# JubSteven/POEM-v2

Hardware: AMD Instinct MI355X
Metric: samples/sec (multi-view frames) POEM-medium 8-view (higher is better)
Workload: dtype f32

## Files before the change

poem-v2_amd/csrc/decoder.cpp:

```cpp
#include "engine.h"

int build_anchor_tables(poem_handle_t h, Plan& p, hipStream_t s, bool at_create) {
  const poem_config_t& c = h->cfg;
  const int C = c.embed, Q = c.nquery;
  const bool ov = !at_create && h->overlap && h->bps_stream && h->knn_stream;
  hipStream_t sk = ov ? h->knn_stream : s;
  if (ov) {
    HIPCHK(hipEventRecord(h->ev_fork0, s));
    HIPCHK(hipStreamWaitEvent(sk, h->ev_fork0, 0));
  }
  const int bb0 = h->block_base(0);
  HIPCHK(poem_launch_canon_xyz(h->tmpl, p.canon_xyz, Q * 3, c.radius, sk));
  for (int k = 0; k < 2; ++k) {
    const int vb = bb0 + (k == 0 ? B_VS : B_VC);
    HIPCHK(poem_launch_vector_attention_tables(p.canon_xyz, h->anchor, h->anchor_idx, h->R(vb + 4), h->R(vb + 5),
                                               h->P(vb + 6), h->R(vb + 7), h->fused[0].w[5 + k], p.tab_g[k], p.tab_p[k],
                                               Q, C, sk));
  }
  if (ov) HIPCHK(hipEventRecord(h->ev_tab, sk));
  h->tables_pending = ov;
  return POEM_OK;
}

namespace {

struct DecoderRun {
  poem_handle_t h;
  Plan& p;
  const poem_config_t& c;
  const float *pt_xyz, *pt_feats;
  float *pose_aa, *betas;
  const int B, C, S, Q, BS, BQ;
// ... 251 lines not shown
      const auto& sw = h->split[2 * i];
      HIPCHK(poem_launch_vector_attention_split(xyz, xyz, anchor, idx_s, shared, p.y3, p.y3 + C, p.y3 + 2 * C, Q, h->R(vsb + 4),
                                                h->R(vsb + 5), sw.w[0], h->R(vsb + 7), sw.w[1], sw.w[2], sw.scales, p.rs, B, Q, C,
                                                3 * C, 3 * C, 3 * C, s));
    } else if (tables && i == 0) {
      if (ov && h->tables_pending) HIPCHK(hipStreamWaitEvent(s, h->ev_tab, 0));
      if (anchor_from_y3)
        HIPCHK(poem_launch_vector_attention_anchored(h->anchor_idx, p.y3, p.y3 + C, p.y3 + 2 * C, Q, h->P(vsb + 10), p.tab_g[0], p.tab_p[0],
                                                     p.rs, B, Q, C, 3 * C, 3 * C, 3 * C, s));
      else {
      if (ov) HIPCHK(hipStreamWaitEvent(s, h->ev_xyz[0], 0));
      HIPCHK(poem_launch_vector_attention_anchored(p.ident, p.y3, p.anch_kv[0], p.anch_kv[0] + C, 32, h->P(vsb + 10), p.tab_g[0],
                                                   p.tab_p[0], p.rs, B, Q, C, 3 * C, 2 * C, 2 * C, s));
      }
    } else if (!shared && p.idx_ld != 32) {
      HIPCHK(poem_launch_vector_attention_k(xyz, xyz, idx_s, kq, p.idx_ld, p.y3, p.y3 + C, p.y3 + 2 * C, Q, h->R(vsb + 4), h->R(vsb + 5),
                                            h->P(vsb + 6), h->R(vsb + 7), h->fused[i].w[5], h->R(vsb + 9), h->P(vsb + 10), h->R(vsb + 11),
                                            p.rs, B, Q, C, 3 * C, 3 * C, 3 * C, 1, s));
    } else {
      poem_vecattn_one_query_blocks(h->va_p1);
      poem_vecattn_valid_neighbours(kq);
      const hipError_t ve = poem_launch_vector_attention(xyz, xyz, anchor, idx_s, shared, p.y3, p.y3 + C, p.y3 + 2 * C, Q, h->R(vsb + 4),
                                                         h->R(vsb + 5), h->P(vsb + 6), h->R(vsb + 7), h->fused[i].w[5], h->R(vsb + 9),
                                                         h->P(vsb + 10), h->R(vsb + 11), p.rs, B, Q, C, 3 * C, 3 * C, 3 * C, 1, s);
      poem_vecattn_valid_neighbours(32);
      poem_vecattn_one_query_blocks(0);
      HIPCHK(ve);
    }
    if (const int rc = prof_end(prof, tables && i == 0 ? 1 : 0); rc != POEM_OK) return rc;
    if (chain) {
      ChainArgs cc = chain_args(1);
      cc.x = p.rs; cc.ldx = C;
      cc.w1 = (const float4*)h->P(vsb + 2); cc.b1 = h->R(vsb + 3); cc.res = hidden; cc.ldres = C; cc.res_mod = 0;
      cc.y1 = p.f_self[i]; cc.ldy1 = C;
      cc.w2 = (const float4*)h->fused[i].w[4]; cc.b2 = h->fused[i].b[4]; cc.n2 = 1; cc.y2 = p.qc; cc.ldy2 = C;
      HIPCHK(poem_launch_chain(&cc, C, s));
      return POEM_OK;
    }
    if (const int rc = gemm(p.rs, C, vsb + 2, vsb + 3, hidden, C, p.f_self[i], C, BQ, C, C, POEM_ACT_NONE); rc != POEM_OK) return rc;
    HIPCHK(poem_launch_gemm(p.f_self[i], C, h->fused[i].w[4], h->fused[i].b[4], nullptr, 0, p.qc, C, BQ, C, C, POEM_ACT_NONE, s));
    return POEM_OK;
// ... 8 lines not shown
        bps_waited[k] = true;
      }
    const bool prof = prof_begin();
    const int kc = shared ? 32 : c.knn;
    if (h->precision != POEM_PRECISION_FP32) {
      if (kc != 32) return POEM_E_UNSUPPORTED;
      const auto& sw = h->split[2 * i + 1];
      HIPCHK(poem_launch_vector_attention_split(xyz, pt_xyz_rows, anchor, idx_c, shared, p.qc, p.y1[i] + 4 * (size_t)BSP * C,
                                                p.y1[i] + 5 * (size_t)BSP * C, SP, h->R(vcb + 4), h->R(vcb + 5), sw.w[0],
                                                h->R(vcb + 7), sw.w[1], sw.w[2], sw.scales, p.rc, B, Q, C, C, C, C, s));
    } else if (tables && i == 0) {
      if (ov) HIPCHK(hipStreamWaitEvent(s, h->ev_xyz[0], 0));
      HIPCHK(poem_launch_vector_attention_anchored(p.ident, p.qc, p.anch_kv[1], p.anch_kv[1] + C, 32, h->P(vcb + 10), p.tab_g[1],
                                                   p.tab_p[1], p.rc, B, Q, C, C, 2 * C, 2 * C, s));
    } else if (!shared && p.idx_ld != 32) {
      HIPCHK(poem_launch_vector_attention_k(xyz, pt_xyz_rows, idx_c, kc, p.idx_ld, p.qc, p.y1[i] + 4 * (size_t)BSP * C, p.y1[i] + 5 * (size_t)BSP * C,
                                            SP, h->R(vcb + 4), h->R(vcb + 5), h->P(vcb + 6), h->R(vcb + 7), h->fused[i].w[6], h->R(vcb + 9),
                                            h->P(vcb + 10), h->R(vcb + 11), p.rc, B, Q, C, C, C, C, 1, s));
    } else {
      poem_vecattn_one_query_blocks(h->va_p1);
      poem_vecattn_valid_neighbours(kc);
      const hipError_t ve = poem_launch_vector_attention(xyz, pt_xyz_rows, anchor, idx_c, shared, p.qc, p.y1[i] + 4 * (size_t)BSP * C,
                                                         p.y1[i] + 5 * (size_t)BSP * C, SP, h->R(vcb + 4), h->R(vcb + 5), h->P(vcb + 6),
                                                         h->R(vcb + 7), h->fused[i].w[6], h->R(vcb + 9), h->P(vcb + 10), h->R(vcb + 11), p.rc, B,
                                                         Q, C, C, C, C, 1, s);
      poem_vecattn_valid_neighbours(32);
      poem_vecattn_one_query_blocks(0);
      HIPCHK(ve);
    }
    return prof_end(prof, tables && i == 0 ? 1 : 0);
  }

  int parametric_tail(int i) {
    const int bb = h->block_base(i);
    HIPCHK(poem_launch_q3_flatten(feats, h->R(bb + B_FLAT_W), h->R(bb + B_FLAT_B), p.q3t, B, Q, C, s));
    HIPCHK(poem_launch_narrow_linear(p.q3t, C, h->R(bb + B_MANO_W), h->R(bb + B_MANO_B), nullptr, p.par, B, C, 106, s));
    HIPCHK(poem_launch_rot6d_to_aa(p.par, pose_aa, betas, B, s));
    if (h->mano_table) HIPCHK(poem_launch_mano_lbs(pose_aa, betas, h->mano_table, p.mano_verts, p.mano_joints, B, h->mano_center, s));
    return POEM_OK;
  }

  int tail(int i, bool* done) {
// ... 92 lines not shown
```

poem-v2_amd/csrc/engine.h:

```cpp
#pragma once
#include "../../include/poem_hip.h"
#include "launchers.h"

#include <hip/hip_runtime.h>

#include <algorithm>
#include <cstdio>
#include <cstdlib>
#include <cstring>
#include <map>
#include <string>
#include <vector>

extern thread_local int g_last_hip_error;

#define HIPCHK(expr)                                 \
  do {                                               \
    (void)hipGetLastError();                         \
    hipError_t e_ = (expr);                          \
    if (e_ != hipSuccess) {                          \
      g_last_hip_error = (int)e_;                    \
      return POEM_E_LAUNCH;                          \
    }                                                \
  } while (0)
// ... 86 lines not shown
  int group_min_views = 0;
  const float* mano_table = nullptr;
  int mano_center = 9;
  int knn_query = 0;
  int knn_fma = 0;
  int chain_tile = 0;
  bool tables_cached = true;
  bool tables_pending = false;
  float* tab_mem = nullptr;
  float *c_canon_xyz = nullptr, *c_tab_g[2] = {}, *c_tab_p[2] = {};
  float* c_qeqp0 = nullptr;
  hipEvent_t ev_bps[8] = {}, ev_xyz[8] = {}, ev_knn[8] = {}, ev_def[8] = {};
  int bps_defer = 0;
  bool f1_split = true;
  int va_p1 = -1;
  int d2_first = 1;
  int wait_merge = -1;
  bool overlap = true;
  static constexpr int IDX_CAP = 32768;
  int32_t* idx_dev = nullptr;
  std::vector<int32_t> idx_host;
  int block_base(int b) const { return T_HEAD_COUNT + b * (cfg.parametric ? B_COUNT_PARAM : B_COUNT); }
  const float* R(int idx) const { return raw[idx]; }
  const void* P(int idx) const { return packed[idx]; }
};

struct Arena {
  char* base;
  size_t off = 0;
  explicit Arena(void* b) : base((char*)b) {}
// ... 43 lines not shown
```

poem-v2_amd/csrc/forward.cpp:

```cpp
#include "engine.h"

namespace {

struct SplitContext {
  bool set = false;
  explicit SplitContext(poem_handle_t h) {
    if (h->precision != POEM_PRECISION_SPLIT_F16X3_ALL) return;
    set = true;
    poem_gemm_split_context(h->packed_base, h->packed_size, h->gemm_split, h->gemm_scales);
    poem_cross_attention_split(1);
    const int dh = h->cfg.embed / h->cfg.heads;
    poem_gemm_split_images(dh == 32 || dh == 64);
  }
  ~SplitContext() {
    if (!set) return;
    poem_gemm_split_context(nullptr, 0, nullptr, nullptr);
    poem_cross_attention_split(0);
    poem_gemm_split_images(0);
  }
};

struct HeadRun {
  poem_handle_t h;
  const poem_config_t& c;
// ... 144 lines not shown
    return POEM_OK;
  }

  int body(hipStream_t st, float* pose_dst, float* betas_dst) {
    if (const int rc = sampling(st); rc != POEM_OK) return rc;
    if (prof_fe) HIPCHK(hipEventRecord(h->prof_ev[2 * prof_slot + 1], st));
    if (!(h->anchor_tables && h->precision == POEM_PRECISION_FP32 && (h->small_batch & 1)))
      HIPCHK(poem_launch_broadcast(h->R(T_QEMB), p.feats0, (long)Q * C, B, st));
    return run_decoder(h, p, p.feats0, p.pt_xyz, p.bps_feat, B, pose_dst, betas_dst, st, true);
  }

  int replay(void* workspace, float* pose_aa, float* betas) {
    if (!h->graphs || h->graph_broken || h->prof_on || h->tables_pending || !h->cap_stream) return 0;
    const std::vector<int64_t> key = {B, plan_views, fused_fe ? -1 : BN, (int64_t)(uintptr_t)workspace, h->precision, h->anchor_tables, h->chains,
                                      h->fused_sampling, h->tables_first, h->chain_combine, h->knn_early, h->overlap, h->chain_tile,
                                      h->tables_cached, h->knn_fma, h->knn_query, h->taps, c.parametric, h->xattn_merge, h->small_batch, h->bps_defer, poem_process_switches(), h->f1_split, h->va_p1, h->group_min_views, h->group_xcd, h->d2_first, h->wait_merge,
                                      (int64_t)(uintptr_t)h->mano_table, h->mano_center};
    poem_handle_s::GraphEntry* hit = nullptr;
    for (auto& g : h->graph_cache)
      if (g.key == key) { hit = &g; break; }
    if (!hit) {
      if (!h->graph_eager) {
        bool seen = false;
        for (auto& k : h->graph_seen) seen = seen || k == key;
        if (!seen) {
          if (h->graph_seen.size() >= 64) h->graph_seen.erase(h->graph_seen.begin());
          h->graph_seen.push_back(key);
          return 0;
        }
      }
      hipGraph_t graph = nullptr;
// ... 139 lines not shown
```

poem-v2_amd/csrc/handle.cpp:

```cpp
#include "engine.h"

#include <atomic>
thread_local int g_last_hip_error = 0;

static std::atomic<int> g_proc_switches{15};
int poem_process_switches() { return g_proc_switches.load(); }

#include <mutex>
namespace {
struct CaptureKit {
  hipStream_t cap = nullptr, bps = nullptr, knn = nullptr;
  hipEvent_t ev[5 + 32] = {};
};
std::mutex g_pool_mutex;
std::map<int, std::vector<CaptureKit>> g_kit_pool;
struct ParkedExec { hipGraphExec_t exec; uint64_t shape; int device; hipEvent_t done; };
std::vector<ParkedExec> g_parked_execs;
std::map<int, std::vector<hipEvent_t>> g_idle_done_events;
int64_t g_exec_reuses = 0, g_exec_update_failures = 0, g_exec_busy_skips = 0;

hipEvent_t done_event_locked(hipStream_t last_stream, bool launched, int device, bool* ok) {
  *ok = true;
  if (!launched) return nullptr;
  int cur = -1;
// ... 469 lines not shown
  else if (k == "knn_fma") h->knn_fma = value != 0;
  else if (k == "knn_query") {
    if (value < 0 || value > 64 || value > h->cfg.nquery) return POEM_E_ARG;
    if (h->precision != POEM_PRECISION_FP32 && value != 0 && value != 32) return POEM_E_UNSUPPORTED;
    h->knn_query = value;
  }
  else if (k == "graphs") h->graphs = value != 0;
  else if (k == "graph_eager") h->graph_eager = value != 0;
  else if (k == "gemm_xcd_map") { poem_gemm_xcd_map(value != 0); g_proc_switches.fetch_and(~1); g_proc_switches.fetch_or(value ? 1 : 0); }
  else if (k == "f1_split") h->f1_split = value != 0;
  else if (k == "xattn_half") { poem_cross_attention_half(value != 0); g_proc_switches.fetch_and(~4); g_proc_switches.fetch_or(value ? 4 : 0); }
  else if (k == "xattn_tail") { poem_cross_attention_tail_halves(value != 0); g_proc_switches.fetch_and(~8); g_proc_switches.fetch_or(value ? 8 : 0); }
  else if (k == "wait_merge") { if (value < -1 || value > 7) return POEM_E_ARG; h->wait_merge = value; }
  else if (k == "d2_first") { if (value < 0 || value > 1) return POEM_E_ARG; h->d2_first = value; }
  else if (k == "va_p1") { if (value < -1 || value > 2) return POEM_E_ARG; h->va_p1 = value; }
  else if (k == "gemm_kslab") { poem_gemm_kslab(value != 0); g_proc_switches.fetch_and(~2); g_proc_switches.fetch_or(value ? 2 : 0); }
  else if (k == "small_batch") h->small_batch = value;
  else if (k == "group_xcd") h->group_xcd = value != 0;
  else if (k == "group_min_views") { if (value < -1) return POEM_E_ARG; h->group_min_views = value; }
  else if (k == "bps_defer") { if (value < 0 || value > 3) return POEM_E_ARG; h->bps_defer = value; }
  else if (k == "chain_tile") { if (value < 0 || value > 3) return POEM_E_ARG; h->chain_tile = value; }
  else return POEM_E_ARG;
  return POEM_OK;
}

int poem_graph_stats(poem_handle_t h, int64_t* out, int n) {
  if (!h || !out || n < 9) return POEM_E_ARG;
  out[0] = (int64_t)h->graph_cache.size();
  out[1] = h->graph_captures; out[2] = h->graph_instantiations; out[3] = h->graph_replays; out[4] = h->plain_forwards;
  out[5] = h->layout_uploads;
// ... 96 lines not shown
```

poem-v2_amd/csrc/launchers.h:

```cpp
#pragma once
#include <hip/hip_runtime.h>

#include "chain.h"
#include "loss.h"
#include "merge.h"

extern "C" {
hipError_t poem_launch_pack_linear(const float* w, int N, int K, void* out, hipStream_t s);
hipError_t poem_launch_gemm(const float* X, int ldx, const void* Wp, const float* bias, const float* R, int ldr,
                            float* Y, int ldy, int M, int N, int K, int act, hipStream_t s);
hipError_t poem_launch_gemm2(const float* X, int ldx, const void* Wp, const float* bias, const float* R, int ldr,
                             float* Y, int ldy, int M, int N, int K, int act, int in_pa, int out_pa, hipStream_t s);
hipError_t poem_launch_unpack_rows(const void* pa, int N, int K, float* out, hipStream_t s);
hipError_t poem_launch_layernorm(const float* x, const float* g, const float* b, float* y, int rows, int cols,
                                 float eps, hipStream_t s);
hipError_t poem_launch_narrow_linear(const float* x, int ldx, const float* w, const float* b, const float* base,
                                     float* out, int rows, int K, int N, hipStream_t s);
hipError_t poem_launch_sine_pe(float* out, int F, int H, int W, int max_views, int normalize, hipStream_t s);
hipError_t poem_launch_frustum_features(const float* intr, const float* extr, float* out, int views, int H, int W, int D, int lid,
                                        double depth_start, double depth_end, const double* position_range, int img0, int img1,
                                        hipStream_t s);
hipError_t poem_launch_conv1x1_ex(const float* feat, const void* Wp, const float* bias, const float* table, const int* pe_index,
                                  float* x, float* xt, int views, int K, int C, int hw, int relu, hipStream_t s);
int poem_sample_merge_supported(int C, int S, int hw);
// ... 68 lines not shown
void poem_cross_attention_split(int on);
void poem_cross_attention_masked_form(int on);
void poem_cross_attention_half(int on);
void poem_cross_attention_tail_halves(int on);
int poem_cross_attention_merges(int NK, int C, int heads);
int poem_cross_attention_fits(int B, int NK, int C);
hipError_t poem_launch_cross_attention_merged_rm(const float* q, const float* k, const float* v, float* ctx, int B, int NQ, int NK,
                                                 int C, int heads, float* scratch, hipStream_t s);
hipError_t poem_launch_cross_attention_merged(const float* q, int ldq, int q_batch_rows, const void* kimg, const void* vimg, float* ctx,
                                              int B, int NQ, int NK, int C, int heads, hipStream_t s);
int poem_gemm_split_applies(const void* Wp, int M, int ldx, int K);
void poem_gemm_split_images(int on);
void poem_gemm_xcd_map(int on);
void poem_gemm_kslab(int on);
void poem_vecattn_one_query_blocks(int on);
void poem_vecattn_valid_neighbours(int k);
hipError_t poem_launch_vector_attention_split(const float* query_xyz, const float* src_xyz, const float* anchor_xyz,
                                              const int* idx, int shared_idx, const float* q, const float* k,
                                              const float* v, int nsrc, const float* wd1, const float* bd1,
                                              const void* wd2, const float* bd2, const void* wg1, const void* wg2,
                                              const float* scales, float* out, int B, int Q, int C, int ldq,
                                              int ldk, int ldv, hipStream_t s);
hipError_t poem_launch_dlt(const float* uv, const float* intr, const float* mat, const int* offs, float* out, int B, int J,
                           int invert, hipStream_t s);
hipError_t poem_launch_dlt_confidence(const float* uv, const float* conf, const float* intr, const float* mat,
                                      const int* offs, float* out, int* sel_count, int B, int J, int invert, int mode,
                                      double threshold, hipStream_t s);
hipError_t poem_launch_pa_epe(const float* pred, const float* gt, float* out, int B, int P, hipStream_t s);
hipError_t poem_launch_pck_accumulate(const float* pred, const float* gt, int B, int P, double vmin, double vmax, int steps,
                                      unsigned int* counts, double* sum, unsigned int* n, float* dist_out, hipStream_t s);
// ... 78 lines not shown
```

poem-v2_amd/csrc/vecattn.hip:

```cpp
#include "common.h"
#ifndef POEM_VA_XCD_SAMPLES
#define POEM_VA_XCD_SAMPLES 1
#endif
#include <algorithm>
#include <cstdlib>

#ifdef POEM_VA_DBG
__device__ long long va_dbg[64 * 4 * 8];
#define VA_STAMP(k) do { if (item >= 6000 && item < 6064 && lane == 0) va_dbg[((item - 6000) * 4 + wv) * 8 + (k)] = clock64(); } while (0)
#else
#define VA_STAMP(k) do { } while (0)
#endif

struct VecAttnArgs {
  const float* query_xyz;
  const float* src_xyz;
  const float* anchor_xyz;
  const int* idx;
  int shared_idx;
  const float* q;
  const float* k;
  const float* v;
  int NS;
  const float* wd1;
// ... 80 lines not shown
  for (int kc = 2; kc < KC; kc += 2) {
    VA_LOADW(a1, kc + 1)
    __builtin_amdgcn_sched_barrier(0);
    VA_CHUNK4(a0, kc, false)
    VA_LOADW(a0, kc + 2)
    __builtin_amdgcn_sched_barrier(0);
    VA_CHUNK4(a1, kc + 1, false)
  }
  }
#undef VA_CHUNK4
#undef VA_LOADW
#undef VA_READX
#undef VA_MMA
}

template <int C, int P, int NW, int MINW, bool COMP, int MODE = 0>
__global__ __launch_bounds__(NW * 64, MINW) void vecattn_kernel(VecAttnArgs A) {
  static_assert(MODE == 0 || MODE == 4 || COMP, "table modes exist for the composed form only");
  constexpr bool MASK = MODE == 3;
  constexpr bool WIDE = MODE == 4;
  constexpr int NTILE = C / 32;
  constexpr int TPW = C / 32 / NW;
  constexpr int XS = 32 * P;
  constexpr int NT = NW * 64;
  extern __shared__ __attribute__((aligned(16))) float smem[];
  float* X = smem;
  float* dl = smem + C * XS;
  int* sidx = reinterpret_cast<int*>(dl + P * 32 * 3);
  int* voffs = sidx + P * 32;
  float* qs = reinterpret_cast<float*>(voffs + P * 32);

  const int tid = threadIdx.x, lane = tid & 63, wv = tid >> 6, j = lane & 31, h = lane >> 5;
  const int groups = (A.Q + P - 1) / P;
// ... 54 lines not shown
      dl[tid * 3 + 0] = qx[0] - nx[0];
      dl[tid * 3 + 1] = qx[1] - nx[1];
      dl[tid * 3 + 2] = qx[2] - nx[2];
    }
#endif
    sidx[tid] = id;
    voffs[tid] = (int)((unsigned)id * (unsigned)(A.ldv * 4));
  }
  if (MODE != 1)
  for (int f = tid; f < P * C / 4; f += NT) {
    const int p = f / (C / 4), c4 = f % (C / 4);
    const int qi = min(i0 + p, A.Q - 1);
    reinterpret_cast<float4*>(qs)[f] = *reinterpret_cast<const float4*>(A.q + ((size_t)b * A.Q + qi) * A.ldq + 4 * c4);
  }
  __syncthreads();
  if (MODE != 2) {
    float db0[P], db1[P];
#pragma unroll
    for (int p = 0; p < P; ++p) {
      db0[p] = dl[(p * 32 + j) * 3 + h];
      db1[p] = h == 0 ? dl[(p * 32 + j) * 3 + 2] : 0.f;
    }
#pragma unroll
    for (int tp = 0; tp < TPW; ++tp) {
      const int crow = (wv * TPW + tp) * 32 + j;
      const float wa0 = A.wd1[crow * 3 + h];
      const float wa1 = h == 0 ? A.wd1[crow * 3 + 2] : 0.f;
      const int cbase = (wv * TPW + tp) * 32 + 4 * h;
#pragma unroll
      for (int p = 0; p < P; ++p) {
        f32x16 hh = zero16();
        hh = mfma32(wa0, db0[p], hh);
        hh = mfma32(wa1, db1[p], hh);
#pragma unroll
        for (int g = 0; g < 4; ++g) {
          const float4 bb = *reinterpret_cast<const float4*>(A.bd1 + cbase + 8 * g);
#pragma unroll
          for (int e = 0; e < 4; e += 2) {
            const int i = 4 * g + e;
            const f32x2 v = f32x2{hh[i], hh[i + 1]} + f32x2{(&bb.x)[e], (&bb.x)[e + 1]};
            X[((wv * TPW + tp) * 32 + mfma_row(i, h)) * XS + 32 * p + j] = fmaxf(v[0], 0.f);
            X[((wv * TPW + tp) * 32 + mfma_row(i + 1, h)) * XS + 32 * p + j] = fmaxf(v[1], 0.f);
          }
        }
      }
    }
    __syncthreads();
  }

  f32x16 acc[TPW][P], pos[TPW][P];

  if (MODE != 1)
#pragma unroll
  for (int tp = 0; tp < TPW; ++tp) {
    const int cbase = (wv * TPW + tp) * 32 + 4 * h;
#pragma unroll
    for (int p = 0; p < P; ++p) {
      const float* krow = A.k + ((size_t)b * A.NS + sidx[p * 32 + j]) * A.ldk + cbase;
#pragma unroll
      for (int g = 0; g < 4; ++g) {
        const float4 kk = *reinterpret_cast<const float4*>(krow + 8 * g);
#pragma unroll
        for (int e = 0; e < 4; ++e) (COMP ? acc : pos)[tp][p][4 * g + e] = (&kk.x)[e];
      }
    }
  }
  __builtin_amdgcn_sched_barrier(0);

  VA_STAMP(1);
  if (MODE == 2) {
    const float4* tg = A.tab_g + ((size_t)ig * NTILE + wv * TPW) * (P * 4 * 64) + lane;
    const float4* tq = A.tab_p + ((size_t)ig * NTILE + wv * TPW) * (P * 4 * 64) + lane;
    float4 gf[TPW][P][4];
#pragma unroll
    for (int tp = 0; tp < TPW; ++tp)
#pragma unroll
      for (int p = 0; p < P; ++p)
#pragma unroll
        for (int g = 0; g < 4; ++g) gf[tp][p][g] = tg[((tp * P + p) * 4 + g) * 64];
#pragma unroll
    for (int tp = 0; tp < TPW; ++tp)
// ... 13 lines not shown
#pragma unroll
        for (int p = 0; p < P; ++p) {
          const float4 qq = *reinterpret_cast<const float4*>(qs + p * C + cbase + 8 * g);
#pragma unroll
          for (int e = 0; e < 4; e += 2) {
            const int i = 4 * g + e;
            const f32x2 tv = (f32x2{(&qq.x)[e], (&qq.x)[e + 1]} - f32x2{acc[tp][p][i], acc[tp][p][i + 1]}) +
                             f32x2{(&gf[tp][p][g].x)[e], (&gf[tp][p][g].x)[e + 1]};
            X[((wv * TPW + tp) * 32 + mfma_row(i, h)) * XS + 32 * p + j] = fmaxf(tv[0], 0.f);
            X[((wv * TPW + tp) * 32 + mfma_row(i + 1, h)) * XS + 32 * p + j] = fmaxf(tv[1], 0.f);
          }
        }
    }
    __syncthreads();
  } else if (COMP) {
    chain_gemm<C, P, NW, TPW, true>(A.wd2, X, pos, wv, lane);
    VA_STAMP(2);
#pragma unroll
    for (int tp = 0; tp < TPW; ++tp) {
      const float bch = A.bd2[(wv * TPW + tp) * 32 + j];
      const f32x2 bb2 = {bch, bch};
#pragma unroll
      for (int p = 0; p < P; ++p)
#pragma unroll
        for (int i = 0; i < 16; i += 2) {
          const f32x2 pv = f32x2{pos[tp][p][i], pos[tp][p][i + 1]} + bb2;
          pos[tp][p][i] = pv[0]; pos[tp][p][i + 1] = pv[1];
        }
    }
    if (MODE != 1) {
#pragma unroll
      for (int tp = 0; tp < TPW; ++tp) {
        const int cbase = (wv * TPW + tp) * 32 + 4 * h;
#pragma unroll
        for (int g = 0; g < 4; ++g)
#pragma unroll
          for (int p = 0; p < P; ++p) {
            const float4 qq = *reinterpret_cast<const float4*>(qs + p * C + cbase + 8 * g);
#pragma unroll
            for (int e = 0; e < 4; e += 2) {
              const int i = 4 * g + e;
              const f32x2 tv = f32x2{(&qq.x)[e], (&qq.x)[e + 1]} - f32x2{acc[tp][p][i], acc[tp][p][i + 1]};
              acc[tp][p][i] = tv[0]; acc[tp][p][i + 1] = tv[1];
            }
          }
      }
    }
    VA_STAMP(3);
    chain_gemm<C, P, NW, TPW, false, MODE == 1>(A.wg1, X, acc, wv, lane);
    VA_STAMP(4);
    __syncthreads();
    if (MODE == 1) {
      float4* tg = A.tab_g + ((size_t)ig * NTILE + wv * TPW) * (P * 4 * 64) + lane;
      float4* tq = A.tab_p + ((size_t)ig * NTILE + wv * TPW) * (P * 4 * 64) + lane;
#pragma unroll
      for (int tp = 0; tp < TPW; ++tp)
#pragma unroll
        for (int p = 0; p < P; ++p)
#pragma unroll
          for (int g = 0; g < 4; ++g) {
            tg[((tp * P + p) * 4 + g) * 64] = float4{acc[tp][p][4 * g], acc[tp][p][4 * g + 1], acc[tp][p][4 * g + 2], acc[tp][p][4 * g + 3]};
            tq[((tp * P + p) * 4 + g) * 64] = float4{pos[tp][p][4 * g], pos[tp][p][4 * g + 1], pos[tp][p][4 * g + 2], pos[tp][p][4 * g + 3]};
          }
      continue;
// ... 134 lines not shown
          const float so = __builtin_amdgcn_exp2f(__builtin_fmaf(wmx[q], k2, nm)), sn = __builtin_amdgcn_exp2f(__builtin_fmaf(mx, k2, nm));
          wsum[q] = __builtin_fmaf(wsum[q], so, sum * sn);
          wres[q] = __builtin_fmaf(wres[q], so, res * sn);
          wmx[q] = m;
        }
        if (ch == nch - 1 && h == 0 && i0 + p < A.Q) A.out[((size_t)b * A.Q + i0 + p) * C + cch] = wres[q] * __builtin_amdgcn_rcpf(wsum[q]);
      } else if (h == 0 && i0 + p < A.Q) A.out[((size_t)b * A.Q + i0 + p) * C + cch] = res * __builtin_amdgcn_rcpf(sum);
    }
  }
  if constexpr (WIDE)
    if (++ch < nch) goto va_chunk;
#undef VA_GATHER
  VA_STAMP(7);
  }
}

template <int C, int P, int NW, int MINW, bool COMP, int MODE = 0>
static hipError_t launch_va_t(const VecAttnArgs& a, hipStream_t s) {
  const int groups = (a.Q + P - 1) / P;
  size_t lds = (size_t)C * 32 * P * 4 + P * 32 * 3 * 4 + 2 * P * 32 * 4 + (size_t)P * C * 4;
#ifdef POEM_VA_DBG
  if (const char* e = getenv("POEM_VA_LDSPAD")) lds += atoi(e);
#endif
  auto kern = vecattn_kernel<C, P, NW, MINW, COMP, MODE>;
  static std::atomic<unsigned long long> optin{0};
  if (hipError_t e = poem_optin_lds(reinterpret_cast<const void*>(kern), lds, optin); e != hipSuccess) return e;
  unsigned grid = (unsigned)(a.B * groups);
  if (a.stagger > 0) {
    grid = std::min(grid, (unsigned)(2 * poem_device_cus()));
  }
  hipLaunchKernelGGL(kern, dim3(grid), dim3(NW * 64), lds, s, a);
  return hipGetLastError();
}

template <int C, int P, int NW, int MINW>
static hipError_t launch_va(const VecAttnArgs& a, hipStream_t s, int mode = 0) {
  if (mode == 4) return a.composed ? launch_va_t<C, P, NW, MINW, true, 4>(a, s) : launch_va_t<C, P, NW, MINW, false, 4>(a, s);
  if (mode == 1) return launch_va_t<C, P, NW, MINW, true, 1>(a, s);
  if (mode == 2) return launch_va_t<C, P, NW, MINW, true, 2>(a, s);
  if (mode == 3) return a.composed ? launch_va_t<C, P, NW, MINW, true, 3>(a, s) : hipErrorInvalidValue;
  return a.composed ? launch_va_t<C, P, NW, MINW, true>(a, s) : launch_va_t<C, P, NW, MINW, false>(a, s);
}

static thread_local int g_va_kvalid = 32;
extern "C" void poem_vecattn_valid_neighbours(int k) { g_va_kvalid = k; }

static thread_local int g_va_p1 = 0;
extern "C" void poem_vecattn_one_query_blocks(int on) { g_va_p1 = on; }

static int va_group_size(int C) { return C == 128 ? 4 : (C >= 512 ? 1 : 2); }

static hipError_t dispatch_va(const VecAttnArgs& a, int C, hipStream_t s, int mode) {
  if (mode != 1 && (unsigned long long)a.NS * a.ldv * 4 + (unsigned long long)C * 4 > (1ull << 31)) return hipErrorInvalidValue;
  if (mode == 4 && (a.kvalid < 1 || a.kvalid > 64 || a.ldidx < a.kvalid || a.shared_idx || a.anchor_xyz)) return hipErrorInvalidValue;
  if (mode == 0 && a.kvalid != 32) {
    if (a.kvalid < 1 || a.kvalid > 32) return hipErrorInvalidValue;
    mode = 3;
  }
  switch (C) {
    case 32: return launch_va<32, 2, 1, 1>(a, s, mode);
    case 64: return launch_va<64, 2, 2, 1>(a, s, mode);
    case 128: return launch_va<128, 4, 4, 2>(a, s, mode);
    case 256: {
      const int g_va_p1 = ::g_va_p1 >= 0 ? ::g_va_p1 : ((long)a.B * a.Q <= 16L * poem_device_cus() ? 1 : 0);
      if (mode == 0 && g_va_p1 == 1 && a.composed) return launch_va_t<256, 1, 4, 3, true>(a, s);
      if (mode == 0 && g_va_p1 == 2 && a.composed) return launch_va_t<256, 1, 4, 2, true>(a, s);
      return launch_va<256, 2, 4, 2>(a, s, mode);
    }
    case 512: return launch_va<512, 1, 4, 2>(a, s, mode);
    case 1024: return launch_va<1024, 1, 8, 2>(a, s, mode);
    default: return hipErrorInvalidValue;
  }
}

extern "C" size_t poem_vector_attention_table_floats(int Q, int C) {
  const int P = va_group_size(C);
  return (size_t)((Q + P - 1) / P) * P * 32 * C;
}

extern "C" hipError_t poem_launch_vector_attention_tables(const float* query_xyz, const float* anchor_xyz, const int* idx,
                                                          const float* wd1, const float* bd1, const void* wd2,
// ... 54 lines not shown
```

poem-v2_amd/hip.py:

```python
import ctypes
import os
import subprocess

import numpy as np
import torch

_HERE = os.path.dirname(os.path.abspath(__file__))
CSRC = os.path.join(_HERE, "csrc")
LIB_PATH = os.environ.get("POEM_HIP_LIB") or os.path.join(CSRC, "libpoem_hip.so")
ASSETS = os.path.join(_HERE, "assets")

ACT_NONE, ACT_RELU, ACT_GELU = 0, 1, 2
PRECISIONS = {"fp32": 0, "split_f16x3": 1, "split_f16x3_all": 2}


class PoemConfig(ctypes.Structure):
    _fields_ = [("embed", ctypes.c_int32), ("in_channels", ctypes.c_int32), ("nsample", ctypes.c_int32),
                ("nquery", ctypes.c_int32), ("heads", ctypes.c_int32), ("nblocks", ctypes.c_int32),
                ("knn", ctypes.c_int32), ("parametric", ctypes.c_int32), ("feat_h", ctypes.c_int32),
                ("feat_w", ctypes.c_int32), ("max_views", ctypes.c_int32), ("radius", ctypes.c_float),
                ("ln_eps", ctypes.c_float),
                ("pe_normalize", ctypes.c_int32), ("petr_embedding", ctypes.c_int32), ("depth_num", ctypes.c_int32),
                ("lid", ctypes.c_int32), ("reserved0", ctypes.c_int32), ("depth_start", ctypes.c_double),
                ("depth_end", ctypes.c_double), ("position_range", ctypes.c_double * 6)]
# ... 452 lines not shown
    if nk is not None:
        assert idx.dim() == 3 and idx.stride(-1) == 1 and idx.stride(1) == idx.shape[2] and anchor_xyz is None
        check(lib().poem_vector_attention_k(ptr(query_xyz), ptr(src_xyz), idx.data_ptr(), int(nk), idx.shape[2], ptr(q), ptr(k),
                                            ptr(v), k.shape[1], ptr(wd1), ptr(bd1), wd2p.data_ptr(), ptr(bd2), wg1p.data_ptr(),
                                            ptr(bg1), wg2p.data_ptr(), ptr(bg2), ptr(out), B, NQ, C, stream()),
              "poem_vector_attention_k")
        return out
    shared = 1 if idx.dim() == 1 else 0
    check(lib().poem_vector_attention(ptr(query_xyz), ptr(src_xyz), ptr(anchor_xyz), idx.data_ptr(), shared, ptr(q), ptr(k),
                                      ptr(v), k.shape[1], ptr(wd1), ptr(bd1), wd2p.data_ptr(), ptr(bd2), wg1p.data_ptr(),
                                      ptr(bg1), wg2p.data_ptr(), ptr(bg2), ptr(out), B, NQ, C, stream()),
          "poem_vector_attention")
    return out



def gemm_split(x, w, bias=None, residual=None, act=ACT_NONE):
    N, K = w.shape
    M = x.shape[0]
    nt = (N + 31) // 32
    img = torch.empty(nt * 32 * K * 4, dtype=torch.uint8, device=w.device)
    sc = torch.empty(nt, dtype=torch.float32, device=w.device)
    check(lib().poem_pack_split_gemm(ptr(w), N, K, img.data_ptr(), sc.data_ptr(), stream()), "poem_pack_split_gemm")
    y = torch.empty(M, N, dtype=torch.float32, device=w.device)
    check(lib().poem_gemm_split(ptr(x), x.stride(0), img.data_ptr(), sc.data_ptr(), ptr(bias), ptr(residual),
                                residual.stride(0) if residual is not None else 0, ptr(y), N, M, N, K, act, stream()),
          "poem_gemm_split")
    return y


# ... 36 lines not shown
```

Baseline: 1469.

## Fuse vector-attention GEMM 1 and GEMM 2 into one pipelined weight pass

Adds a chain_gemm12 routine that computes the position-encoding GEMM (wd2) and the gating GEMM (wg1) in a single k-loop. It shares the X operand reads and keeps a 2- or 4-deep ring of register-prefetched weight chunks. The K gather, wd1 and bias loads are hoisted ahead of the loop, and the q-k subtraction now runs before the fused GEMM. This removes a second pass over the LDS activations and overlaps the weight loads with the MFMAs, at the cost of more registers, which can lower occupancy. The path is on by default through a new va_fuse12 switch, and the switch is added to the graph cache key.

```diff
diff --git a/poem-v2_amd/csrc/decoder.cpp b/poem-v2_amd/csrc/decoder.cpp
--- a/poem-v2_amd/csrc/decoder.cpp
+++ b/poem-v2_amd/csrc/decoder.cpp
@@ -13,9 +13,12 @@
   HIPCHK(poem_launch_canon_xyz(h->tmpl, p.canon_xyz, Q * 3, c.radius, sk));
   for (int k = 0; k < 2; ++k) {
     const int vb = bb0 + (k == 0 ? B_VS : B_VC);
-    HIPCHK(poem_launch_vector_attention_tables(p.canon_xyz, h->anchor, h->anchor_idx, h->R(vb + 4), h->R(vb + 5),
-                                               h->P(vb + 6), h->R(vb + 7), h->fused[0].w[5 + k], p.tab_g[k], p.tab_p[k],
-                                               Q, C, sk));
+    const int fuse_was = poem_vecattn_fused_pass(h->va_fuse12);
+    const hipError_t te = poem_launch_vector_attention_tables(p.canon_xyz, h->anchor, h->anchor_idx, h->R(vb + 4), h->R(vb + 5),
+                                                              h->P(vb + 6), h->R(vb + 7), h->fused[0].w[5 + k], p.tab_g[k], p.tab_p[k],
+                                                              Q, C, sk);
+    poem_vecattn_fused_pass(fuse_was);
+    HIPCHK(te);
   }
   if (ov) HIPCHK(hipEventRecord(h->ev_tab, sk));
   h->tables_pending = ov;
@@ -297,17 +300,22 @@
                                                    p.tab_p[0], p.rs, B, Q, C, 3 * C, 2 * C, 2 * C, s));
       }
     } else if (!shared && p.idx_ld != 32) {
-      HIPCHK(poem_launch_vector_attention_k(xyz, xyz, idx_s, kq, p.idx_ld, p.y3, p.y3 + C, p.y3 + 2 * C, Q, h->R(vsb + 4), h->R(vsb + 5),
-                                            h->P(vsb + 6), h->R(vsb + 7), h->fused[i].w[5], h->R(vsb + 9), h->P(vsb + 10), h->R(vsb + 11),
-                                            p.rs, B, Q, C, 3 * C, 3 * C, 3 * C, 1, s));
+      const int fuse_was = poem_vecattn_fused_pass(h->va_fuse12);
+      const hipError_t ve = poem_launch_vector_attention_k(xyz, xyz, idx_s, kq, p.idx_ld, p.y3, p.y3 + C, p.y3 + 2 * C, Q, h->R(vsb + 4),
+                                                           h->R(vsb + 5), h->P(vsb + 6), h->R(vsb + 7), h->fused[i].w[5], h->R(vsb + 9),
+                                                           h->P(vsb + 10), h->R(vsb + 11), p.rs, B, Q, C, 3 * C, 3 * C, 3 * C, 1, s);
+      poem_vecattn_fused_pass(fuse_was);
+      HIPCHK(ve);
     } else {
       poem_vecattn_one_query_blocks(h->va_p1);
+      const int fuse_was = poem_vecattn_fused_pass(h->va_fuse12);
       poem_vecattn_valid_neighbours(kq);
       const hipError_t ve = poem_launch_vector_attention(xyz, xyz, anchor, idx_s, shared, p.y3, p.y3 + C, p.y3 + 2 * C, Q, h->R(vsb + 4),
                                                          h->R(vsb + 5), h->P(vsb + 6), h->R(vsb + 7), h->fused[i].w[5], h->R(vsb + 9),
                                                          h->P(vsb + 10), h->R(vsb + 11), p.rs, B, Q, C, 3 * C, 3 * C, 3 * C, 1, s);
       poem_vecattn_valid_neighbours(32);
       poem_vecattn_one_query_blocks(0);
+      poem_vecattn_fused_pass(fuse_was);
       HIPCHK(ve);
     }
     if (const int rc = prof_end(prof, tables && i == 0 ? 1 : 0); rc != POEM_OK) return rc;
@@ -346,11 +354,16 @@
       HIPCHK(poem_launch_vector_attention_anchored(p.ident, p.qc, p.anch_kv[1], p.anch_kv[1] + C, 32, h->P(vcb + 10), p.tab_g[1],
                                                    p.tab_p[1], p.rc, B, Q, C, C, 2 * C, 2 * C, s));
     } else if (!shared && p.idx_ld != 32) {
-      HIPCHK(poem_launch_vector_attention_k(xyz, pt_xyz_rows, idx_c, kc, p.idx_ld, p.qc, p.y1[i] + 4 * (size_t)BSP * C, p.y1[i] + 5 * (size_t)BSP * C,
-                                            SP, h->R(vcb + 4), h->R(vcb + 5), h->P(vcb + 6), h->R(vcb + 7), h->fused[i].w[6], h->R(vcb + 9),
-                                            h->P(vcb + 10), h->R(vcb + 11), p.rc, B, Q, C, C, C, C, 1, s));
+      const int fuse_was = poem_vecattn_fused_pass(h->va_fuse12);
+      const hipError_t ve = poem_launch_vector_attention_k(xyz, pt_xyz_rows, idx_c, kc, p.idx_ld, p.qc, p.y1[i] + 4 * (size_t)BSP * C,
+                                                           p.y1[i] + 5 * (size_t)BSP * C, SP, h->R(vcb + 4), h->R(vcb + 5), h->P(vcb + 6),
+                                                           h->R(vcb + 7), h->fused[i].w[6], h->R(vcb + 9), h->P(vcb + 10), h->R(vcb + 11), p.rc,
+                                                           B, Q, C, C, C, C, 1, s);
+      poem_vecattn_fused_pass(fuse_was);
+      HIPCHK(ve);
     } else {
       poem_vecattn_one_query_blocks(h->va_p1);
+      const int fuse_was = poem_vecattn_fused_pass(h->va_fuse12);
       poem_vecattn_valid_neighbours(kc);
       const hipError_t ve = poem_launch_vector_attention(xyz, pt_xyz_rows, anchor, idx_c, shared, p.qc, p.y1[i] + 4 * (size_t)BSP * C,
                                                          p.y1[i] + 5 * (size_t)BSP * C, SP, h->R(vcb + 4), h->R(vcb + 5), h->P(vcb + 6),
@@ -358,6 +371,7 @@
                                                          Q, C, C, C, C, 1, s);
       poem_vecattn_valid_neighbours(32);
       poem_vecattn_one_query_blocks(0);
+      poem_vecattn_fused_pass(fuse_was);
       HIPCHK(ve);
     }
     return prof_end(prof, tables && i == 0 ? 1 : 0);
diff --git a/poem-v2_amd/csrc/engine.h b/poem-v2_amd/csrc/engine.h
--- a/poem-v2_amd/csrc/engine.h
+++ b/poem-v2_amd/csrc/engine.h
@@ -124,6 +124,7 @@
   int bps_defer = 0;
   bool f1_split = true;
   int va_p1 = -1;
+  int va_fuse12 = 1;
   int d2_first = 1;
   int wait_merge = -1;
   bool overlap = true;
diff --git a/poem-v2_amd/csrc/forward.cpp b/poem-v2_amd/csrc/forward.cpp
--- a/poem-v2_amd/csrc/forward.cpp
+++ b/poem-v2_amd/csrc/forward.cpp
@@ -182,7 +182,7 @@
     if (!h->graphs || h->graph_broken || h->prof_on || h->tables_pending || !h->cap_stream) return 0;
     const std::vector<int64_t> key = {B, plan_views, fused_fe ? -1 : BN, (int64_t)(uintptr_t)workspace, h->precision, h->anchor_tables, h->chains,
                                       h->fused_sampling, h->tables_first, h->chain_combine, h->knn_early, h->overlap, h->chain_tile,
-                                      h->tables_cached, h->knn_fma, h->knn_query, h->taps, c.parametric, h->xattn_merge, h->small_batch, h->bps_defer, poem_process_switches(), h->f1_split, h->va_p1, h->group_min_views, h->group_xcd, h->d2_first, h->wait_merge,
+                                      h->tables_cached, h->knn_fma, h->knn_query, h->taps, c.parametric, h->xattn_merge, h->small_batch, h->bps_defer, poem_process_switches(), h->f1_split, h->va_p1, h->va_fuse12, h->group_min_views, h->group_xcd, h->d2_first, h->wait_merge,
                                       (int64_t)(uintptr_t)h->mano_table, h->mano_center};
     poem_handle_s::GraphEntry* hit = nullptr;
     for (auto& g : h->graph_cache)
diff --git a/poem-v2_amd/csrc/handle.cpp b/poem-v2_amd/csrc/handle.cpp
--- a/poem-v2_amd/csrc/handle.cpp
+++ b/poem-v2_amd/csrc/handle.cpp
@@ -507,6 +507,7 @@
   else if (k == "wait_merge") { if (value < -1 || value > 7) return POEM_E_ARG; h->wait_merge = value; }
   else if (k == "d2_first") { if (value < 0 || value > 1) return POEM_E_ARG; h->d2_first = value; }
   else if (k == "va_p1") { if (value < -1 || value > 2) return POEM_E_ARG; h->va_p1 = value; }
+  else if (k == "va_fuse12") { if (value < 0 || value > 1) return POEM_E_ARG; h->va_fuse12 = value; }
   else if (k == "gemm_kslab") { poem_gemm_kslab(value != 0); g_proc_switches.fetch_and(~2); g_proc_switches.fetch_or(value ? 2 : 0); }
   else if (k == "small_batch") h->small_batch = value;
   else if (k == "group_xcd") h->group_xcd = value != 0;
diff --git a/poem-v2_amd/csrc/launchers.h b/poem-v2_amd/csrc/launchers.h
--- a/poem-v2_amd/csrc/launchers.h
+++ b/poem-v2_amd/csrc/launchers.h
@@ -106,6 +106,7 @@
 void poem_gemm_xcd_map(int on);
 void poem_gemm_kslab(int on);
 void poem_vecattn_one_query_blocks(int on);
+int poem_vecattn_fused_pass(int on);
 void poem_vecattn_valid_neighbours(int k);
 hipError_t poem_launch_vector_attention_split(const float* query_xyz, const float* src_xyz, const float* anchor_xyz,
                                               const int* idx, int shared_idx, const float* q, const float* k,
diff --git a/poem-v2_amd/csrc/vecattn.hip b/poem-v2_amd/csrc/vecattn.hip
--- a/poem-v2_amd/csrc/vecattn.hip
+++ b/poem-v2_amd/csrc/vecattn.hip
@@ -1,6 +1,9 @@
 #include "common.h"
 #ifndef POEM_VA_XCD_SAMPLES
 #define POEM_VA_XCD_SAMPLES 1
+#endif
+#ifndef POEM_VA_RING256
+#define POEM_VA_RING256 4
 #endif
 #include <algorithm>
 #include <cstdlib>
@@ -118,9 +121,134 @@
 #undef VA_MMA
 }
 
-template <int C, int P, int NW, int MINW, bool COMP, int MODE = 0>
+template <int C, int P, int NW, int TPW, int RING, bool ZERO_ACC>
+__device__ __forceinline__ void chain_gemm12(const float4* __restrict__ Wd, const float4* __restrict__ Wg,
+                                             const float* __restrict__ X, f32x16 (&pos)[TPW][P], f32x16 (&acc)[TPW][P],
+                                             int wv, int lane) {
+  constexpr int KC = C / 8;
+  constexpr int XS = 32 * P;
+  static_assert(RING == 2 || RING == 4, "weight rings of two or four chunks");
+  static_assert(KC % RING == 0, "C must be a multiple of 8 x the ring depth");
+  const int j = lane & 31, h = lane >> 5;
+  const __amdgpu_buffer_rsrc_t drs = frag_rsrc(Wd, (unsigned)(C * C * 4));
+  const __amdgpu_buffer_rsrc_t grs = frag_rsrc(Wg, (unsigned)(C * C * 4));
+  const int wbase = __builtin_amdgcn_readfirstlane(wv) * TPW * KC * 1024;
+  const int loff = lane * 16;
+  const float* xc = X + (4 * h) * XS + j;
+#define VA_LOADW(D, G, KCI)                                                               \
+  {                                                                                       \
+    const int kq_ = min((KCI), KC - 1);                                                   \
+    _Pragma("unroll") for (int tp = 0; tp < TPW; ++tp) {                                  \
+      D[tp] = frag_load(drs, loff, wbase + (tp * KC + kq_) * 1024);                       \
+      G[tp] = frag_load(grs, loff, wbase + (tp * KC + kq_) * 1024);                       \
+    }                                                                                     \
+  }
+#define VA_READX(XR, KCI, T)                                                              \
+  {                                                                                       \
+    const int kq_ = min((KCI), KC - 1);                                                   \
+    _Pragma("unroll") for (int p = 0; p < P; ++p) XR[p] = xc[(kq_ * 8 + (T)) * XS + 32 * p]; \
+  }
+#define VA_MMA(D, G, T, XR, INIT)                                                         \
+  _Pragma("unroll") for (int tp = 0; tp < TPW; ++tp) {                                    \
+    const float dv = (&D[tp].x)[T], gv = (&G[tp].x)[T];                                   \
+    _Pragma("unroll") for (int p = 0; p < P; ++p)                                         \
+      pos[tp][p] = mfma32(XR[p], dv, (INIT) ? zero16() : pos[tp][p]);                     \
+    _Pragma("unroll") for (int p = 0; p < P; ++p)                                         \
+      acc[tp][p] = mfma32(gv, XR[p], (INIT) && ZERO_ACC ? zero16() : acc[tp][p]);         \
+  }
+  float x0[P], x1[P], x2[P], x3[P];
+#define VA_CHUNK4(D, G, KCI, INIT)                                                          \
+  VA_MMA(D, G, 0, x0, INIT) __builtin_amdgcn_sched_barrier(0); VA_READX(x0, (KCI) + 1, 0) __builtin_amdgcn_sched_barrier(0);  \
+  VA_MMA(D, G, 1, x1, false) __builtin_amdgcn_sched_barrier(0); VA_READX(x1, (KCI) + 1, 1) __builtin_amdgcn_sched_barrier(0); \
+  VA_MMA(D, G, 2, x2, false) __builtin_amdgcn_sched_barrier(0); VA_READX(x2, (KCI) + 1, 2) __builtin_amdgcn_sched_barrier(0); \
+  VA_MMA(D, G, 3, x3, false) __builtin_amdgcn_sched_barrier(0); VA_READX(x3, (KCI) + 1, 3) __builtin_amdgcn_sched_barrier(0);
+  float4 d0[TPW], d1[TPW], g0[TPW], g1[TPW];
+  if constexpr (RING == 4) {
+  float4 d2[TPW], d3[TPW], g2[TPW], g3[TPW];
+  VA_LOADW(d0, g0, 0)
+  VA_READX(x0, 0, 0) VA_READX(x1, 0, 1) VA_READX(x2, 0, 2) VA_READX(x3, 0, 3)
+  VA_LOADW(d1, g1, 1)
+  VA_LOADW(d2, g2, 2)
+  __builtin_amdgcn_sched_barrier(0);
+#define VA_GROUP(KC0, INIT)                                                                           \
+  VA_LOADW(d3, g3, (KC0) + 3) __builtin_amdgcn_sched_barrier(0); VA_CHUNK4(d0, g0, (KC0), INIT)       \
+  VA_LOADW(d0, g0, (KC0) + 4) __builtin_amdgcn_sched_barrier(0); VA_CHUNK4(d1, g1, (KC0) + 1, false)  \
+  VA_LOADW(d1, g1, (KC0) + 5) __builtin_amdgcn_sched_barrier(0); VA_CHUNK4(d2, g2, (KC0) + 2, false)  \
+  VA_LOADW(d2, g2, (KC0) + 6) __builtin_amdgcn_sched_barrier(0); VA_CHUNK4(d3, g3, (KC0) + 3, false)
+  VA_GROUP(0, true)
+  for (int kc = 4; kc < KC; kc += 4) { VA_GROUP(kc, false) }
+#undef VA_GROUP
+  } else {
+  VA_LOADW(d0, g0, 0)
+  VA_READX(x0, 0, 0) VA_READX(x1, 0, 1) VA_READX(x2, 0, 2) VA_READX(x3, 0, 3)
+  VA_LOADW(d1, g1, 1)
+  __builtin_amdgcn_sched_barrier(0);
+  VA_CHUNK4(d0, g0, 0, true)
+  VA_LOADW(d0, g0, 2)
+  __builtin_amdgcn_sched_barrier(0);
+  VA_CHUNK4(d1, g1, 1, false)
+  for (int kc = 2; kc < KC; kc += 2) {
+    VA_LOADW(d1, g1, kc + 1)
+    __builtin_amdgcn_sched_barrier(0);
+    VA_CHUNK4(d0, g0, kc, false)
+    VA_LOADW(d0, g0, kc + 2)
+    __builtin_amdgcn_sched_barrier(0);
+    VA_CHUNK4(d1, g1, kc + 1, false)
+  }
+  }
+#undef VA_CHUNK4
+#undef VA_LOADW
+#undef VA_READX
+#undef VA_MMA
+}
+
+template <int C, int P, int NW, int MINW, int MODE>
+constexpr int va_fuse_ring() {
+  if (C <= 128) return 4;
+  if (C == 256 && P == 2) return MODE == 4 ? 0 : POEM_VA_RING256;
+  if (C == 256 && P == 1) return MINW == 3 ? 2 : 4;
+  return 0;
+}
+
+#define VA_GATHER_K(DST)                                                                             \
+  _Pragma("unroll") for (int tp = 0; tp < TPW; ++tp) {                                               \
+    const int cbase = (wv * TPW + tp) * 32 + 4 * h;                                                  \
+    _Pragma("unroll") for (int p = 0; p < P; ++p) {                                                  \
+      const float* krow = A.k + ((size_t)b * A.NS + sidx[p * 32 + j]) * A.ldk + cbase;               \
+      _Pragma("unroll") for (int g = 0; g < 4; ++g) {                                                \
+        const float4 kk = *reinterpret_cast<const float4*>(krow + 8 * g);                            \
+        _Pragma("unroll") for (int e = 0; e < 4; ++e) DST[tp][p][4 * g + e] = (&kk.x)[e];            \
+      }                                                                                              \
+    }                                                                                                \
+  }
+#define VA_ADD_BD2                                                                                   \
+  _Pragma("unroll") for (int tp = 0; tp < TPW; ++tp) {                                               \
+    const float bch = A.bd2[(wv * TPW + tp) * 32 + j];                                               \
+    const f32x2 bb2 = {bch, bch};                                                                    \
+    _Pragma("unroll") for (int p = 0; p < P; ++p)                                                    \
+      _Pragma("unroll") for (int i = 0; i < 16; i += 2) {                                            \
+        const f32x2 pv = f32x2{pos[tp][p][i], pos[tp][p][i + 1]} + bb2;                              \
+        pos[tp][p][i] = pv[0]; pos[tp][p][i + 1] = pv[1];                                            \
+      }                                                                                              \
+  }
+#define VA_SUB_QK                                                                                    \
+  _Pragma("unroll") for (int tp = 0; tp < TPW; ++tp) {                                               \
+    const int cbase = (wv * TPW + tp) * 32 + 4 * h;                                                  \
+    _Pragma("unroll") for (int g = 0; g < 4; ++g)                                                    \
+      _Pragma("unroll") for (int p = 0; p < P; ++p) {                                                \
+        const float4 qq = *reinterpret_cast<const float4*>(qs + p * C + cbase + 8 * g);              \
+        _Pragma("unroll") for (int e = 0; e < 4; e += 2) {                                           \
+          const int i = 4 * g + e;                                                                   \
+          const f32x2 tv = f32x2{(&qq.x)[e], (&qq.x)[e + 1]} - f32x2{acc[tp][p][i], acc[tp][p][i + 1]}; \
+          acc[tp][p][i] = tv[0]; acc[tp][p][i + 1] = tv[1];                                          \
+        }                                                                                            \
+      }                                                                                              \
+  }
+
+template <int C, int P, int NW, int MINW, bool COMP, int MODE = 0, int FUSE = 0>
 __global__ __launch_bounds__(NW * 64, MINW) void vecattn_kernel(VecAttnArgs A) {
   static_assert(MODE == 0 || MODE == 4 || COMP, "table modes exist for the composed form only");
+  static_assert(FUSE == 0 || (COMP && MODE != 2), "the one-pass form is the composed GEMM 1 + GEMM 2");
   constexpr bool MASK = MODE == 3;
   constexpr bool WIDE = MODE == 4;
   constexpr int NTILE = C / 32;
@@ -205,6 +333,22 @@
     reinterpret_cast<float4*>(qs)[f] = *reinterpret_cast<const float4*>(A.q + ((size_t)b * A.Q + qi) * A.ldq + 4 * c4);
   }
   __syncthreads();
+  f32x16 acc[TPW][P], pos[TPW][P];
+  float wd1a[TPW], wd1b[TPW];
+  float4 bd1v[TPW][4];
+  if constexpr (FUSE != 0) {
+#pragma unroll
+    for (int tp = 0; tp < TPW; ++tp) {
+      const int crow = (wv * TPW + tp) * 32 + j;
+      wd1a[tp] = A.wd1[crow * 3 + h];
+      wd1b[tp] = h == 0 ? A.wd1[crow * 3 + 2] : 0.f;
+#pragma unroll
+      for (int g = 0; g < 4; ++g) bd1v[tp][g] = *reinterpret_cast<const float4*>(A.bd1 + (wv * TPW + tp) * 32 + 4 * h + 8 * g);
+    }
+    __builtin_amdgcn_sched_barrier(0);
+    if (MODE != 1) VA_GATHER_K(acc)
+    __builtin_amdgcn_sched_barrier(0);
+  }
   if (MODE != 2) {
     float db0[P], db1[P];
 #pragma unroll
@@ -215,8 +359,8 @@
 #pragma unroll
     for (int tp = 0; tp < TPW; ++tp) {
       const int crow = (wv * TPW + tp) * 32 + j;
-      const float wa0 = A.wd1[crow * 3 + h];
-      const float wa1 = h == 0 ? A.wd1[crow * 3 + 2] : 0.f;
+      const float wa0 = FUSE != 0 ? wd1a[tp] : A.wd1[crow * 3 + h];
+      const float wa1 = FUSE != 0 ? wd1b[tp] : (h == 0 ? A.wd1[crow * 3 + 2] : 0.f);
       const int cbase = (wv * TPW + tp) * 32 + 4 * h;
 #pragma unroll
       for (int p = 0; p < P; ++p) {
@@ -225,7 +369,7 @@
         hh = mfma32(wa1, db1[p], hh);
 #pragma unroll
         for (int g = 0; g < 4; ++g) {
-          const float4 bb = *reinterpret_cast<const float4*>(A.bd1 + cbase + 8 * g);
+          const float4 bb = FUSE != 0 ? bd1v[tp][g] : *reinterpret_cast<const float4*>(A.bd1 + cbase + 8 * g);
 #pragma unroll
           for (int e = 0; e < 4; e += 2) {
             const int i = 4 * g + e;
@@ -239,23 +383,7 @@
     __syncthreads();
   }
 
-  f32x16 acc[TPW][P], pos[TPW][P];
-
-  if (MODE != 1)
-#pragma unroll
-  for (int tp = 0; tp < TPW; ++tp) {
-    const int cbase = (wv * TPW + tp) * 32 + 4 * h;
-#pragma unroll
-    for (int p = 0; p < P; ++p) {
-      const float* krow = A.k + ((size_t)b * A.NS + sidx[p * 32 + j]) * A.ldk + cbase;
-#pragma unroll
-      for (int g = 0; g < 4; ++g) {
-        const float4 kk = *reinterpret_cast<const float4*>(krow + 8 * g);
-#pragma unroll
-        for (int e = 0; e < 4; ++e) (COMP ? acc : pos)[tp][p][4 * g + e] = (&kk.x)[e];
-      }
-    }
-  }
+  if (MODE != 1 && FUSE == 0) VA_GATHER_K((COMP ? acc : pos))
   __builtin_amdgcn_sched_barrier(0);
 
   VA_STAMP(1);
@@ -299,40 +427,19 @@
     }
     __syncthreads();
   } else if (COMP) {
+    if constexpr (FUSE != 0) {
+      if (MODE != 1) VA_SUB_QK
+      VA_STAMP(3);
+      chain_gemm12<C, P, NW, TPW, FUSE, MODE == 1>(A.wd2, A.wg1, X, pos, acc, wv, lane);
+      VA_ADD_BD2
+    } else {
     chain_gemm<C, P, NW, TPW, true>(A.wd2, X, pos, wv, lane);
     VA_STAMP(2);
-#pragma unroll
-    for (int tp = 0; tp < TPW; ++tp) {
-      const float bch = A.bd2[(wv * TPW + tp) * 32 + j];
-      const f32x2 bb2 = {bch, bch};
-#pragma unroll
-      for (int p = 0; p < P; ++p)
-#pragma unroll
-        for (int i = 0; i < 16; i += 2) {
-          const f32x2 pv = f32x2{pos[tp][p][i], pos[tp][p][i + 1]} + bb2;
-          pos[tp][p][i] = pv[0]; pos[tp][p][i + 1] = pv[1];
-        }
-    }
-    if (MODE != 1) {
-#pragma unroll
-      for (int tp = 0; tp < TPW; ++tp) {
-        const int cbase = (wv * TPW + tp) * 32 + 4 * h;
-#pragma unroll
-        for (int g = 0; g < 4; ++g)
-#pragma unroll
-          for (int p = 0; p < P; ++p) {
-            const float4 qq = *reinterpret_cast<const float4*>(qs + p * C + cbase + 8 * g);
-#pragma unroll
-            for (int e = 0; e < 4; e += 2) {
-              const int i = 4 * g + e;
-              const f32x2 tv = f32x2{(&qq.x)[e], (&qq.x)[e + 1]} - f32x2{acc[tp][p][i], acc[tp][p][i + 1]};
-              acc[tp][p][i] = tv[0]; acc[tp][p][i + 1] = tv[1];
-            }
-          }
-      }
-    }
+    VA_ADD_BD2
+    if (MODE != 1) VA_SUB_QK
     VA_STAMP(3);
     chain_gemm<C, P, NW, TPW, false, MODE == 1>(A.wg1, X, acc, wv, lane);
+    }
     VA_STAMP(4);
     __syncthreads();
     if (MODE == 1) {
@@ -497,15 +604,18 @@
   VA_STAMP(7);
   }
 }
-
-template <int C, int P, int NW, int MINW, bool COMP, int MODE = 0>
+#undef VA_GATHER_K
+#undef VA_ADD_BD2
+#undef VA_SUB_QK
+
+template <int C, int P, int NW, int MINW, bool COMP, int MODE = 0, int FUSE = 0>
 static hipError_t launch_va_t(const VecAttnArgs& a, hipStream_t s) {
   const int groups = (a.Q + P - 1) / P;
   size_t lds = (size_t)C * 32 * P * 4 + P * 32 * 3 * 4 + 2 * P * 32 * 4 + (size_t)P * C * 4;
 #ifdef POEM_VA_DBG
   if (const char* e = getenv("POEM_VA_LDSPAD")) lds += atoi(e);
 #endif
-  auto kern = vecattn_kernel<C, P, NW, MINW, COMP, MODE>;
+  auto kern = vecattn_kernel<C, P, NW, MINW, COMP, MODE, FUSE>;
   static std::atomic<unsigned long long> optin{0};
   if (hipError_t e = poem_optin_lds(reinterpret_cast<const void*>(kern), lds, optin); e != hipSuccess) return e;
   unsigned grid = (unsigned)(a.B * groups);
@@ -516,13 +626,27 @@
   return hipGetLastError();
 }
 
+static thread_local int g_va_fuse12 = 1;
+extern "C" int poem_vecattn_fused_pass(int on) {
+  const int was = g_va_fuse12;
+  g_va_fuse12 = on;
+  return was;
+}
+
+template <int C, int P, int NW, int MINW, int MODE>
+static hipError_t launch_va_comp(const VecAttnArgs& a, hipStream_t s) {
+  constexpr int RING = va_fuse_ring<C, P, NW, MINW, MODE>();
+  if (RING != 0 && g_va_fuse12) return launch_va_t<C, P, NW, MINW, true, MODE, RING>(a, s);
+  return launch_va_t<C, P, NW, MINW, true, MODE>(a, s);
+}
+
 template <int C, int P, int NW, int MINW>
 static hipError_t launch_va(const VecAttnArgs& a, hipStream_t s, int mode = 0) {
-  if (mode == 4) return a.composed ? launch_va_t<C, P, NW, MINW, true, 4>(a, s) : launch_va_t<C, P, NW, MINW, false, 4>(a, s);
-  if (mode == 1) return launch_va_t<C, P, NW, MINW, true, 1>(a, s);
+  if (mode == 4) return a.composed ? launch_va_comp<C, P, NW, MINW, 4>(a, s) : launch_va_t<C, P, NW, MINW, false, 4>(a, s);
+  if (mode == 1) return launch_va_comp<C, P, NW, MINW, 1>(a, s);
   if (mode == 2) return launch_va_t<C, P, NW, MINW, true, 2>(a, s);
-  if (mode == 3) return a.composed ? launch_va_t<C, P, NW, MINW, true, 3>(a, s) : hipErrorInvalidValue;
-  return a.composed ? launch_va_t<C, P, NW, MINW, true>(a, s) : launch_va_t<C, P, NW, MINW, false>(a, s);
+  if (mode == 3) return a.composed ? launch_va_comp<C, P, NW, MINW, 3>(a, s) : hipErrorInvalidValue;
+  return a.composed ? launch_va_comp<C, P, NW, MINW, 0>(a, s) : launch_va_t<C, P, NW, MINW, false>(a, s);
 }
 
 static thread_local int g_va_kvalid = 32;
@@ -546,8 +670,8 @@
     case 128: return launch_va<128, 4, 4, 2>(a, s, mode);
     case 256: {
       const int g_va_p1 = ::g_va_p1 >= 0 ? ::g_va_p1 : ((long)a.B * a.Q <= 16L * poem_device_cus() ? 1 : 0);
-      if (mode == 0 && g_va_p1 == 1 && a.composed) return launch_va_t<256, 1, 4, 3, true>(a, s);
-      if (mode == 0 && g_va_p1 == 2 && a.composed) return launch_va_t<256, 1, 4, 2, true>(a, s);
+      if (mode == 0 && g_va_p1 == 1 && a.composed) return launch_va_comp<256, 1, 4, 3, 0>(a, s);
+      if (mode == 0 && g_va_p1 == 2 && a.composed) return launch_va_comp<256, 1, 4, 2, 0>(a, s);
       return launch_va<256, 2, 4, 2>(a, s, mode);
     }
     case 512: return launch_va<512, 1, 4, 2>(a, s, mode);
diff --git a/poem-v2_amd/hip.py b/poem-v2_amd/hip.py
--- a/poem-v2_amd/hip.py
+++ b/poem-v2_amd/hip.py
@@ -490,6 +490,15 @@
     return out
 
 
+_FUSED_PASS = None
+
+
+def vecattn_fused_pass(on):
+    global _FUSED_PASS
+    if _FUSED_PASS is None:
+        _FUSED_PASS = ctypes.CFUNCTYPE(_i, _i)(("poem_vecattn_fused_pass", lib()))
+    return _FUSED_PASS(int(on))
+
 
 def gemm_split(x, w, bias=None, residual=None, act=ACT_NONE):
     N, K = w.shape
```

Result: no change. 1473, median of 6 (+0.3%).
